# kkahatapitiya/Coarse-Fine-Networks

Measured on AMD Instinct MI355X. Metric: clips/sec (fwd+bwd+SGD) x3d_fine X3D-M T=256x224x224, higher is better.
Workload: dtype f32; 1 GPU; x3d_fine X3D-M train step (fwd+loss+bwd+SGD), 8x3x256x224x224 clips per GPU, random-init weights; clips_per_gpu=8, frames=256, parallelism=dp1, launch=eager

## Files before the change

### coarse-fine-networks_amd/csrc/pwfused.hip

```cpp
#include "cfn_common.h"
#include <stdlib.h>

#include "pw_common.h"

typedef float __attribute__((ext_vector_type(4))) pf4;

#define PF_PT 64
#define PF_PITCH 65

struct PfArgs {
    const float* gy; const float* y; const double* gs; const double* gq; const double* gsc;
    const float* w;
    const float* x; const double* pa; const double* pb;
    float* gx; double* gA; double* gB; double* gw;
    const float* acc; int acc_s, acc_Ho, acc_Wo, Hi, Wi, T;
    int N, M, K, Q, nstrips, stages;
};

template <int MTW, int NTW, int ACT>
__global__ __launch_bounds__(256, ACT < 0 ? 3 : 2) void pw_bwd_fused_kernel(const PfArgs a) {
    extern __shared__ __attribute__((aligned(16))) float smem[];
    constexpr bool EPI = ACT >= 0;
    constexpr int ACTV = EPI ? ACT : CFN_ACT_NONE;
    constexpr int BM = 32 * MTW, BN = 32 * NTW;
    constexpr int NG = BM / 16, NX = BN / 16;
    constexpr int NT16 = BN / 16, KS = BM / 4;
    const int tid = threadIdx.x, wave = tid >> 6, lane = tid & 63, half = lane >> 5, col = lane & 31;
    const int m16 = lane & 15, kq = lane >> 4;
    unsigned L = cfn_xcd_remap(blockIdx.x, gridDim.x);
    const int strip = L % a.nstrips;
    const int n = L / a.nstrips;
    const int M = a.M, K = a.K, Q = a.Q;

    constexpr int IMG = (BM + BN) * PF_PITCH;
    float* img0 = smem;
    float* sCg = smem + 2 * IMG;
    float* sCz = sCg + 2 * BM;
    float* sCx = sCz + BM;
    float* sSt = sCx + 2 * BN;
    for (int m = tid; m < BM; m += 256) {
        const bool ok = m < M;
        sCg[2 * m] = (ok && a.gs) ? (float)a.gs[(long)n * M + m] : 0.0f;
        sCg[2 * m + 1] = (ok && a.gq && a.y) ? 2.0f * (float)a.gq[(long)n * M + m] : 0.0f;
        sCz[m] = (ok && a.gsc) ? (float)a.gsc[(long)n * M + m] : 1.0f;
    }
    for (int k = tid; k < BN; k += 256) {
        const bool ok = EPI && k < K;
        sCx[2 * k] = ok ? (float)a.pa[(long)n * K + k] : 1.0f;
        sCx[2 * k + 1] = ok ? (float)a.pb[(long)n * K + k] : 0.0f;
    }
    float wq[NT16][KS];
#pragma unroll
    for (int t = 0; t < NT16; ++t)
#pragma unroll
        for (int s = 0; s < KS; ++s) {
            const int ci = t * 16 + m16, co = 4 * s + kq;
            wq[t][s] = (ci < K && co < M) ? a.w[(long)co * K + ci] : 0.0f;
        }
    float ca[NTW], cb[NTW];
#pragma unroll
    for (int j = 0; j < NTW; ++j) {
        const int k = j * 32 + col;
        const bool ok = EPI && k < K;
        ca[j] = ok ? (float)a.pa[(long)n * K + k] : 1.0f;
        cb[j] = ok ? (float)a.pb[(long)n * K + k] : 0.0f;
    }
    f16v acc[MTW][NTW];
#pragma unroll
    for (int i = 0; i < MTW; ++i)
#pragma unroll
        for (int j = 0; j < NTW; ++j)
#pragma unroll
            for (int r = 0; r < 16; ++r) acc[i][j][r] = 0.0f;
    float sa[NT16][4], sb[NT16][4];
#pragma unroll
    for (int t = 0; t < NT16; ++t)
#pragma unroll
        for (int r = 0; r < 4; ++r) { sa[t][r] = 0.0f; sb[t][r] = 0.0f; }
    __syncthreads();

    const int lrow = tid >> 4, c4 = (tid & 15) * 4;
    constexpr int OOB = 0x7ffffff0;
    __amdgpu_buffer_rsrc_t rg = cfn_rsrc(const_cast<float*>(a.gy + (long)n * M * Q), (unsigned)((long)M * Q * 4));
    __amdgpu_buffer_rsrc_t ry = cfn_rsrc(const_cast<float*>((a.y ? a.y : a.gy) + (long)n * M * Q), a.y ? (unsigned)((long)M * Q * 4) : 0u);
    __amdgpu_buffer_rsrc_t rx = cfn_rsrc(const_cast<float*>(a.x + (long)n * K * Q), (unsigned)((long)K * Q * 4));
    __amdgpu_buffer_rsrc_t rd = cfn_rsrc(a.gx + (long)n * K * Q, (unsigned)((long)K * Q * 4));
    pf4 pg[NG], py[NG], px[NX];
    int vog[NG], vox[NX];
#pragma unroll
    for (int it = 0; it < NG; ++it) vog[it] = (it * 16 + lrow) < M ? ((it * 16 + lrow) * Q + c4) * 4 : OOB;
#pragma unroll
    for (int it = 0; it < NX; ++it) vox[it] = (it * 16 + lrow) < K ? ((it * 16 + lrow) * Q + c4) * 4 : OOB;
    auto prefetch = [&](int q0) {
        const bool inq = q0 + c4 < Q;
#pragma unroll
        for (int it = 0; it < NG; ++it) {
            const int vo = inq ? vog[it] : OOB;
            pg[it] = __builtin_bit_cast(pf4, __builtin_amdgcn_raw_buffer_load_b128(rg, vo, q0 * 4, 0));
            py[it] = __builtin_bit_cast(pf4, __builtin_amdgcn_raw_buffer_load_b128(ry, vo, q0 * 4, 0));
        }
#pragma unroll
        for (int it = 0; it < NX; ++it)
            px[it] = __builtin_bit_cast(pf4, __builtin_amdgcn_raw_buffer_load_b128(rx, inq ? vox[it] : OOB, q0 * 4, 0));
    };
    auto stage = [&](int q0, float* sG, float* sX) {
        const bool inq = q0 + c4 < Q;
#pragma unroll
        for (int it = 0; it < NG; ++it) {
            const int row = it * 16 + lrow;
            const float cs = cfn_settle(sCg[2 * row]), cq = cfn_settle(sCg[2 * row + 1]), cz = cfn_settle(sCz[row]);
            const bool ok = inq && (row < M);
            float* d = sG + row * PF_PITCH + c4;
            d[0] = ok ? fmaf(py[it].x, cq, fmaf(pg[it].x, cz, cs)) : 0.0f;
            d[1] = ok ? fmaf(py[it].y, cq, fmaf(pg[it].y, cz, cs)) : 0.0f;
            d[2] = ok ? fmaf(py[it].z, cq, fmaf(pg[it].z, cz, cs)) : 0.0f;
            d[3] = ok ? fmaf(py[it].w, cq, fmaf(pg[it].w, cz, cs)) : 0.0f;
        }
#pragma unroll
        for (int it = 0; it < NX; ++it) {
            const int row = it * 16 + lrow;
            float* d = sX + row * PF_PITCH + c4;
            d[0] = px[it].x; d[1] = px[it].y; d[2] = px[it].z; d[3] = px[it].w;
        }
    };

    const int qbeg = strip * a.stages * PF_PT;
    const int nst = min(a.stages, (Q - qbeg + PF_PT - 1) / PF_PT);
    if (nst > 0) {
        prefetch(qbeg);
        stage(qbeg, img0, img0 + BM * PF_PITCH);
        if (nst > 1) prefetch(qbeg + PF_PT);
    }
    __syncthreads();
    const int pbase = wave * (PF_PT / 4);
    const int hw = a.Hi * a.Wi;
    const int acc_pitch4 = a.T * a.acc_Ho * a.acc_Wo * 4;
    __amdgpu_buffer_rsrc_t racc = cfn_rsrc(const_cast<float*>(a.acc ? a.acc + (long)n * K * (acc_pitch4 / 4) : a.gy), a.acc ? (unsigned)((long)K * acc_pitch4) : 0u);
    for (int st = 0; st < nst; ++st) {
        const int q0 = qbeg + st * PF_PT;
        float* cur = img0 + (st & 1) * IMG;
        float* nxt = img0 + ((st + 1) & 1) * IMG;
        if (st + 1 < nst) {
            stage(q0 + PF_PT, nxt, nxt + BM * PF_PITCH);
            if (st + 2 < nst) prefetch(q0 + 2 * PF_PT);
        }
        const float* sG = cur;
        const float* sX = cur + BM * PF_PITCH;
#pragma unroll
        for (int s = 0; s < PF_PT / 8; ++s) {
            const int p = pbase + 2 * s + half;
            float av[MTW], bv[NTW];
#pragma unroll
            for (int i = 0; i < MTW; ++i) av[i] = sG[(i * 32 + col) * PF_PITCH + p];
#pragma unroll
            for (int j = 0; j < NTW; ++j) {
                const float xr = sX[(j * 32 + col) * PF_PITCH + p];
                bv[j] = EPI ? cfn_act<ACTV>(fmaf(xr, ca[j], cb[j])) : xr;
            }
#pragma unroll
            for (int i = 0; i < MTW; ++i)
#pragma unroll
                for (int j = 0; j < NTW; ++j) acc[i][j] = __builtin_amdgcn_mfma_f32_32x32x2f32(av[i], bv[j], acc[i][j], 0, 0, 0);
        }
        pf4 da[NT16];
#pragma unroll
        for (int t = 0; t < NT16; ++t) da[t] = (pf4){0.f, 0.f, 0.f, 0.f};
#pragma unroll
        for (int s = 0; s < KS; ++s) {
            const float b = sG[(4 * s + kq) * PF_PITCH + pbase + m16];
#pragma unroll
            for (int t = 0; t < NT16; ++t) da[t] = __builtin_amdgcn_mfma_f32_16x16x4f32(wq[t][s], b, da[t], 0, 0, 0);
        }
        const int q = q0 + pbase + m16;
        const bool qv = q < Q;
        int aoff = OOB;
        if (a.acc && qv) {
            const int tq = q / hw, rq = q - tq * hw;
            const int hq = rq / a.Wi, wq_ = rq - hq * a.Wi;
            if (hq % a.acc_s == 0 && wq_ % a.acc_s == 0) aoff = (((tq * a.acc_Ho + hq / a.acc_s) * a.acc_Wo + wq_ / a.acc_s)) * 4;
        }
        float av4[NT16][4];
#pragma unroll
        for (int t = 0; t < NT16; ++t)
#pragma unroll
            for (int r = 0; r < 4; ++r) av4[t][r] = 0.0f;
        if (a.acc) {
            const unsigned arow = (unsigned)aoff + (unsigned)(4 * kq) * (unsigned)acc_pitch4;
#pragma unroll
            for (int t = 0; t < NT16; ++t)
#pragma unroll
                for (int r = 0; r < 4; ++r)
                    av4[t][r] = __builtin_bit_cast(float, __builtin_amdgcn_raw_buffer_load_b32(
                        racc, (int)(aoff == OOB ? (unsigned)OOB : arow + (unsigned)r * (unsigned)acc_pitch4), t * 16 * acc_pitch4, 0));
        }
#pragma unroll
        for (int t = 0; t < NT16; ++t) {
#pragma unroll
            for (int r = 0; r < 4; ++r) {
                const int ci = t * 16 + 4 * kq + r;
                const bool ok = qv && ci < K;
                float v = da[t][r] + av4[t][r];
                if (EPI) {
                    const float xr = sX[ci * PF_PITCH + pbase + m16];
                    const float pa = sCx[2 * ci], pb = sCx[2 * ci + 1];
                    const float dz = ok ? v * cfn_act_grad<ACTV>(fmaf(xr, pa, pb)) : 0.0f;
                    sa[t][r] = fmaf(dz, xr, sa[t][r]);
                    sb[t][r] += dz;
                    v = dz * pa;
                }
                __builtin_amdgcn_raw_buffer_store_b32(__builtin_bit_cast(unsigned, v), rd, ok ? (ci * Q + pbase + m16) * 4 : OOB, q0 * 4, 0);
            }
        }
        __syncthreads();
    }

    if (EPI) {
#pragma unroll
        for (int t = 0; t < NT16; ++t)
#pragma unroll
            for (int r = 0; r < 4; ++r) {
                float u = sa[t][r], v = sb[t][r];
#pragma unroll
                for (int o = 1; o < 16; o <<= 1) { u += __shfl_xor(u, o, 64); v += __shfl_xor(v, o, 64); }
                if (m16 == 0) {
                    const int ci = t * 16 + 4 * kq + r;
                    sSt[(wave * BN + ci) * 2] = u;
                    sSt[(wave * BN + ci) * 2 + 1] = v;
                }
            }
    }
    constexpr int CWP = BN + 1;
    float* cw = smem + wave * (BM * CWP);
#pragma unroll
    for (int i = 0; i < MTW; ++i)
#pragma unroll
        for (int j = 0; j < NTW; ++j)
#pragma unroll
            for (int r = 0; r < 16; ++r) {
                const int ml = i * 32 + (r & 3) + 8 * (r >> 2) + 4 * half;
                cw[ml * CWP + j * 32 + col] = acc[i][j][r];
            }
    __syncthreads();
    for (int e = tid; e < BM * BN; e += 256) {
        const int ml = e / BN, kl = e - ml * BN;
        const int o = ml * CWP + kl;
        const float v = (smem[o] + smem[BM * CWP + o]) + (smem[2 * BM * CWP + o] + smem[3 * BM * CWP + o]);
        if (ml < M && kl < K) cfn_add64(&a.gw[(long)ml * K + kl], (double)v);
    }
    if (EPI && tid < K) {
        const float u = (sSt[2 * tid] + sSt[(BN + tid) * 2]) + (sSt[(2 * BN + tid) * 2] + sSt[(3 * BN + tid) * 2]);
        const float v = (sSt[2 * tid + 1] + sSt[(BN + tid) * 2 + 1]) + (sSt[(2 * BN + tid) * 2 + 1] + sSt[(3 * BN + tid) * 2 + 1]);
        cfn_add64(&a.gA[(long)n * K + tid], (double)u);
        cfn_add64(&a.gB[(long)n * K + tid], (double)v);
    }
}

template <int MTW, int NTW>
static int pf_launch(const PfArgs& a, int act, bool epi, unsigned blocks, hipStream_t st) {
    constexpr int BM = 32 * MTW, BN = 32 * NTW;
    size_t lds = ((size_t)2 * (BM + BN) * PF_PITCH + 3 * BM + 10 * BN) * sizeof(float);
    const size_t lds_cw = (size_t)4 * BM * (BN + 1) * sizeof(float);
    if (lds_cw > lds) lds = lds_cw;
#define CFN_PF_GO(ACTV)                                                                                         \
    do {                                                                                                        \
        auto k = pw_bwd_fused_kernel<MTW, NTW, ACTV>;                                                           \
        if (lds > 48 * 1024) (void)hipFuncSetAttribute((const void*)k, hipFuncAttributeMaxDynamicSharedMemorySize, (int)lds); \
        hipLaunchKernelGGL(k, dim3(blocks), dim3(256), lds, st, a);                                             \
    } while (0)
    if (!epi) CFN_PF_GO(-1);
    else if (act == CFN_ACT_RELU) CFN_PF_GO(CFN_ACT_RELU);
    else if (act == CFN_ACT_SWISH) CFN_PF_GO(CFN_ACT_SWISH);
    else CFN_PF_GO(CFN_ACT_NONE);
#undef CFN_PF_GO
    return cfn_check_launch("pwconv_bwd_fused");
}

extern "C" int cfn_pwconv_bwd_fused(const float* gy, const float* y, const double* gsum, const double* gsumsq, const float* w,
                                    const float* x, const double* A, const double* B, int act, float* gx, double* gA, double* gB,
                                    double* gw, int N, int Cin, int Cout, int T, int Hi, int Wi, const float* acc, int acc_stride,
                                    const double* gscale, void* stream) {
    CFN_REQUIRE(gy && w && x && gx && gw, "cfn_pwconv_bwd_fused: null tensor");
    CFN_REQUIRE((A == nullptr) == (B == nullptr), "cfn_pwconv_bwd_fused: A/B mismatch");
    CFN_REQUIRE(A == nullptr || (gA && gB), "cfn_pwconv_bwd_fused: prologue needs gA, gB");
    CFN_REQUIRE(gsumsq == nullptr || y != nullptr, "cfn_pwconv_bwd_fused: gsumsq needs y");
    CFN_REQUIRE(acc == nullptr || acc_stride >= 1, "cfn_pwconv_bwd_fused: bad acc_stride");
    {
        const int rs = pwfs_try_launch(gy, y, gsum, gsumsq, w, x, A, B, act, gx, gA, gB, gw, N, Cin, Cout, T, Hi, Wi, acc, acc_stride, gscale, (hipStream_t)stream);
        if (rs != -1) return rs;
    }
    const long Ql = (long)T * Hi * Wi;
    if (Cin > 64 || Cout > 64 || (Cin > 32 && Cout > 32) || Ql % 4 != 0 || Ql >= (1L << 30)) return -1;
    if ((long)Cout * Ql * 4 >= 0x7ffffff0L || (long)Cin * Ql * 4 >= 0x7ffffff0L) return -1;
    if (A && act != CFN_ACT_NONE && act != CFN_ACT_RELU && act != CFN_ACT_SWISH) return -1;
    if ((((uintptr_t)gy | (uintptr_t)x | (uintptr_t)(y ? y : gy)) & 15) != 0) return -1;
    PfArgs a = {};
    a.gy = gy; a.y = gsumsq ? y : nullptr; a.gs = gsum; a.gq = gsumsq; a.gsc = gscale; a.w = w; a.x = x; a.pa = A; a.pb = B;
    a.gx = gx; a.gA = gA; a.gB = gB; a.gw = gw;
    a.acc = acc; a.acc_s = acc ? acc_stride : 1; a.Hi = Hi; a.Wi = Wi; a.T = T;
    a.acc_Ho = (Hi - 1) / a.acc_s + 1; a.acc_Wo = (Wi - 1) / a.acc_s + 1;
    a.N = N; a.M = Cout; a.K = Cin; a.Q = (int)Ql;
    const long nst = cfn_cdiv(Ql, PF_PT);
    const bool epi = A != nullptr;
    long want = (epi ? 1024 : 1536) / N;
    if (want < 1) want = 1;
    long stages = cfn_cdiv(nst, want);
    if (stages < 4) stages = 4;
    a.stages = (int)stages;
    a.nstrips = (int)cfn_cdiv(nst, stages);
    const unsigned blocks = (unsigned)((long)N * a.nstrips);
    hipStream_t st = (hipStream_t)stream;
    CfnProfScope prof(CFN_K_PWCONV_BWD, st, 4.0 * N * ((double)Cout * Ql * (a.y ? 2 : 1) + (double)Cin * Ql * 2));
    if (Cout > 32) return pf_launch<2, 1>(a, act, epi, blocks, st);
    if (Cin > 32) return pf_launch<1, 2>(a, act, epi, blocks, st);
    return pf_launch<1, 1>(a, act, epi, blocks, st);
}
```

Before: 107.0 clips/s.

## Add warp-specialized 512-thread pointwise-conv backward kernel splitting dW and dX waves

Adds a 512-thread variant of the fused pointwise-conv backward kernel. Four waves stage data and accumulate the weight gradient while four other waves compute the input gradient and activation epilogue, with weights held in LDS for wider tiles and the acc loads issued early. It is used for epilogue cases whose tile exceeds 32x32, so the two GEMM-like tasks can overlap on separate waves. Debug knockout switches are compiled in only under a macro. The cost is more LDS and registers per block, extra synchronisation, and lower occupancy per block.

New measurement: 107.5 clips/s, median of 6. About the same (+0.5%).

```diff
diff --git a/coarse-fine-networks_amd/csrc/pwfused.hip b/coarse-fine-networks_amd/csrc/pwfused.hip
--- a/coarse-fine-networks_amd/csrc/pwfused.hip
+++ b/coarse-fine-networks_amd/csrc/pwfused.hip
@@ -15,7 +15,15 @@
     float* gx; double* gA; double* gB; double* gw;
     const float* acc; int acc_s, acc_Ho, acc_Wo, Hi, Wi, T;
     int N, M, K, Q, nstrips, stages;
+#ifdef CFN_PWF_KNOCKOUTS
+    int dbg;
+#endif
 };
+#ifdef CFN_PWF_KNOCKOUTS
+#define PF_DBG(a) ((a).dbg)
+#else
+#define PF_DBG(a) 0
+#endif
 
 template <int MTW, int NTW, int ACT>
 __global__ __launch_bounds__(256, ACT < 0 ? 3 : 2) void pw_bwd_fused_kernel(const PfArgs a) {
@@ -146,6 +154,7 @@
         }
         const float* sG = cur;
         const float* sX = cur + BM * PF_PITCH;
+        if (!(PF_DBG(a) & 1))
 #pragma unroll
         for (int s = 0; s < PF_PT / 8; ++s) {
             const int p = pbase + 2 * s + half;
@@ -165,6 +174,7 @@
         pf4 da[NT16];
 #pragma unroll
         for (int t = 0; t < NT16; ++t) da[t] = (pf4){0.f, 0.f, 0.f, 0.f};
+        if (!(PF_DBG(a) & 2))
 #pragma unroll
         for (int s = 0; s < KS; ++s) {
             const float b = sG[(4 * s + kq) * PF_PITCH + pbase + m16];
@@ -200,7 +210,7 @@
                 const int ci = t * 16 + 4 * kq + r;
                 const bool ok = qv && ci < K;
                 float v = da[t][r] + av4[t][r];
-                if (EPI) {
+                if (EPI && !(PF_DBG(a) & 4)) {
                     const float xr = sX[ci * PF_PITCH + pbase + m16];
                     const float pa = sCx[2 * ci], pb = sCx[2 * ci + 1];
                     const float dz = ok ? v * cfn_act_grad<ACTV>(fmaf(xr, pa, pb)) : 0.0f;
@@ -208,7 +218,7 @@
                     sb[t][r] += dz;
                     v = dz * pa;
                 }
-                __builtin_amdgcn_raw_buffer_store_b32(__builtin_bit_cast(unsigned, v), rd, ok ? (ci * Q + pbase + m16) * 4 : OOB, q0 * 4, 0);
+                __builtin_amdgcn_raw_buffer_store_b32(__builtin_bit_cast(unsigned, v), rd, (ok && !(PF_DBG(a) & 8)) ? (ci * Q + pbase + m16) * 4 : OOB, q0 * 4, 0);
             }
         }
         __syncthreads();
@@ -255,23 +265,334 @@
     }
 }
 
+template <int MTW, int NTW, int ACT>
+__global__ __launch_bounds__(512, 4) void pw_bwd_fused8_kernel(const PfArgs a) {
+    extern __shared__ __attribute__((aligned(16))) float smem[];
+    constexpr bool EPI = ACT >= 0;
+    constexpr int ACTV = EPI ? ACT : CFN_ACT_NONE;
+    constexpr int BM = 32 * MTW, BN = 32 * NTW;
+    constexpr int NG = BM / 16, NX = BN / 16;
+    constexpr int NT16 = BN / 16, KS = BM / 4;
+    constexpr bool WLDS = NT16 > 2;
+    const int tid = threadIdx.x, wave = tid >> 6, lane = tid & 63, half = lane >> 5, col = lane & 31;
+    const int m16 = lane & 15, kq = lane >> 4, w4 = wave & 3;
+    unsigned L = cfn_xcd_remap(blockIdx.x, gridDim.x);
+    const int strip = L % a.nstrips;
+    const int n = L / a.nstrips;
+    const int M = a.M, K = a.K, Q = a.Q;
+
+    constexpr int IMG = (BM + BN) * PF_PITCH;
+    float* img0 = smem;
+    float* sCg = smem + 2 * IMG;
+    float* sCz = sCg + 2 * BM;
+    float* sCx = sCz + BM;
+    float* sSt = sCx + 2 * BN;
+    float* sWt = sSt + 8 * BN;
+    for (int m = tid; m < BM; m += 512) {
+        const bool ok = m < M;
+        sCg[2 * m] = (ok && a.gs) ? (float)a.gs[(long)n * M + m] : 0.0f;
+        sCg[2 * m + 1] = (ok && a.gq && a.y) ? 2.0f * (float)a.gq[(long)n * M + m] : 0.0f;
+        sCz[m] = (ok && a.gsc) ? (float)a.gsc[(long)n * M + m] : 1.0f;
+    }
+    for (int k = tid; k < BN; k += 512) {
+        const bool ok = EPI && k < K;
+        sCx[2 * k] = ok ? (float)a.pa[(long)n * K + k] : 1.0f;
+        sCx[2 * k + 1] = ok ? (float)a.pb[(long)n * K + k] : 0.0f;
+    }
+    __syncthreads();
+
+    constexpr int OOB = 0x7ffffff0;
+    const int qbeg = strip * a.stages * PF_PT;
+    const int nst = min(a.stages, (Q - qbeg + PF_PT - 1) / PF_PT);
+    const int pbase = w4 * (PF_PT / 4);
+    constexpr int CWP = BN + 1;
+
+    if (wave < 4) {
+        float ca[NTW], cb[NTW];
+#pragma unroll
+        for (int j = 0; j < NTW; ++j) {
+            const int k = j * 32 + col;
+            const bool ok = EPI && k < K;
+            ca[j] = ok ? (float)a.pa[(long)n * K + k] : 1.0f;
+            cb[j] = ok ? (float)a.pb[(long)n * K + k] : 0.0f;
+        }
+        f16v acc[MTW][NTW];
+#pragma unroll
+        for (int i = 0; i < MTW; ++i)
+#pragma unroll
+            for (int j = 0; j < NTW; ++j)
+#pragma unroll
+                for (int r = 0; r < 16; ++r) acc[i][j][r] = 0.0f;
+        const int lrow = tid >> 4, c4 = (tid & 15) * 4;
+        __amdgpu_buffer_rsrc_t rg = cfn_rsrc(const_cast<float*>(a.gy + (long)n * M * Q), (unsigned)((long)M * Q * 4));
+        __amdgpu_buffer_rsrc_t ry = cfn_rsrc(const_cast<float*>((a.y ? a.y : a.gy) + (long)n * M * Q), a.y ? (unsigned)((long)M * Q * 4) : 0u);
+        __amdgpu_buffer_rsrc_t rx = cfn_rsrc(const_cast<float*>(a.x + (long)n * K * Q), (unsigned)((long)K * Q * 4));
+        pf4 pg[NG], py[NG], px[NX];
+        const int vo0 = (lrow * Q + c4) * 4, vstep = 16 * Q * 4;
+        auto prefetch_g = [&](int q0) {
+            const bool inq = q0 + c4 < Q;
+#pragma unroll
+            for (int it = 0; it < NG; ++it) {
+                const int vo = (inq && it * 16 + lrow < M) ? vo0 + it * vstep : OOB;
+                pg[it] = __builtin_bit_cast(pf4, __builtin_amdgcn_raw_buffer_load_b128(rg, vo, q0 * 4, 0));
+                py[it] = __builtin_bit_cast(pf4, __builtin_amdgcn_raw_buffer_load_b128(ry, vo, q0 * 4, 0));
+            }
+        };
+        auto prefetch_x = [&](int q0) {
+            const bool inq = q0 + c4 < Q;
+#pragma unroll
+            for (int it = 0; it < NX; ++it)
+                px[it] = __builtin_bit_cast(pf4, __builtin_amdgcn_raw_buffer_load_b128(rx, (inq && it * 16 + lrow < K) ? vo0 + it * vstep : OOB, q0 * 4, 0));
+        };
+        auto stage_g = [&](int q0, float* sG) {
+            const bool inq = q0 + c4 < Q;
+#pragma unroll
+            for (int it = 0; it < NG; ++it) {
+                const int row = it * 16 + lrow;
+                const float cs = cfn_settle(sCg[2 * row]), cq = cfn_settle(sCg[2 * row + 1]), cz = cfn_settle(sCz[row]);
+                const bool ok = inq && (row < M);
+                float* d = sG + row * PF_PITCH + c4;
+                d[0] = ok ? fmaf(py[it].x, cq, fmaf(pg[it].x, cz, cs)) : 0.0f;
+                d[1] = ok ? fmaf(py[it].y, cq, fmaf(pg[it].y, cz, cs)) : 0.0f;
+                d[2] = ok ? fmaf(py[it].z, cq, fmaf(pg[it].z, cz, cs)) : 0.0f;
+                d[3] = ok ? fmaf(py[it].w, cq, fmaf(pg[it].w, cz, cs)) : 0.0f;
+            }
+        };
+        auto stage_x = [&](float* sX) {
+#pragma unroll
+            for (int it = 0; it < NX; ++it) {
+                float* d = sX + (it * 16 + lrow) * PF_PITCH + c4;
+                d[0] = px[it].x; d[1] = px[it].y; d[2] = px[it].z; d[3] = px[it].w;
+            }
+        };
+        if (nst > 0) {
+            prefetch_x(qbeg);
+            prefetch_g(qbeg);
+            stage_x(img0 + BM * PF_PITCH);
+            if (nst > 1) prefetch_x(qbeg + PF_PT);
+            stage_g(qbeg, img0);
+            if (nst > 1) prefetch_g(qbeg + PF_PT);
+        }
+        __syncthreads();
+        for (int st = 0; st < nst; ++st) {
+            const int q0 = qbeg + st * PF_PT;
+            float* cur = img0 + (st & 1) * IMG;
+            float* nxt = img0 + ((st + 1) & 1) * IMG;
+            if (st + 1 < nst) {
+                stage_x(nxt + BM * PF_PITCH);
+                if (st + 2 < nst) prefetch_x(q0 + 2 * PF_PT);
+                stage_g(q0 + PF_PT, nxt);
+                if (st + 2 < nst) prefetch_g(q0 + 2 * PF_PT);
+            }
+            const float* sG = cur;
+            const float* sX = cur + BM * PF_PITCH;
+            if (!(PF_DBG(a) & 1))
+#pragma unroll
+            for (int s = 0; s < PF_PT / 8; ++s) {
+                const int p = pbase + 2 * s + half;
+                float av[MTW], bv[NTW];
+#pragma unroll
+                for (int i = 0; i < MTW; ++i) av[i] = sG[(i * 32 + col) * PF_PITCH + p];
+#pragma unroll
+                for (int j = 0; j < NTW; ++j) {
+                    const float xr = sX[(j * 32 + col) * PF_PITCH + p];
+                    bv[j] = EPI ? cfn_act<ACTV>(fmaf(xr, ca[j], cb[j])) : xr;
+                }
+#pragma unroll
+                for (int i = 0; i < MTW; ++i)
+#pragma unroll
+                    for (int j = 0; j < NTW; ++j) acc[i][j] = __builtin_amdgcn_mfma_f32_32x32x2f32(av[i], bv[j], acc[i][j], 0, 0, 0);
+            }
+            __syncthreads();
+        }
+        float* cw = smem + wave * (BM * CWP);
+#pragma unroll
+        for (int i = 0; i < MTW; ++i)
+#pragma unroll
+            for (int j = 0; j < NTW; ++j)
+#pragma unroll
+                for (int r = 0; r < 16; ++r) {
+                    const int ml = i * 32 + (r & 3) + 8 * (r >> 2) + 4 * half;
+                    cw[ml * CWP + j * 32 + col] = acc[i][j][r];
+                }
+    } else {
+        float wq[WLDS ? 1 : NT16][WLDS ? 1 : KS];
+        if (WLDS) {
+            if (wave == 4) {
+#pragma unroll
+                for (int t = 0; t < NT16; ++t)
+#pragma unroll
+                    for (int s = 0; s < KS; ++s) {
+                        const int ci = t * 16 + m16, co = 4 * s + kq;
+                        sWt[(((s >> 2) * NT16 + t) * 64 + lane) * 4 + (s & 3)] = (ci < K && co < M) ? a.w[(long)co * K + ci] : 0.0f;
+                    }
+            }
+        } else {
+#pragma unroll
+            for (int t = 0; t < NT16; ++t)
+#pragma unroll
+                for (int s = 0; s < KS; ++s) {
+                    const int ci = t * 16 + m16, co = 4 * s + kq;
+                    wq[t][s] = (ci < K && co < M) ? a.w[(long)co * K + ci] : 0.0f;
+                }
+        }
+        float sa[NT16][4], sb[NT16][4];
+#pragma unroll
+        for (int t = 0; t < NT16; ++t)
+#pragma unroll
+            for (int r = 0; r < 4; ++r) { sa[t][r] = 0.0f; sb[t][r] = 0.0f; }
+        __amdgpu_buffer_rsrc_t rd = cfn_rsrc(a.gx + (long)n * K * Q, (unsigned)((long)K * Q * 4));
+        const int hw = a.Hi * a.Wi;
+        const int acc_pitch4 = a.T * a.acc_Ho * a.acc_Wo * 4;
+        __amdgpu_buffer_rsrc_t racc = cfn_rsrc(const_cast<float*>(a.acc ? a.acc + (long)n * K * (acc_pitch4 / 4) : a.gy), a.acc ? (unsigned)((long)K * acc_pitch4) : 0u);
+        auto acc_off = [&](int q0) {
+            const int q = q0 + pbase + m16;
+            int aoff = OOB;
+            if (a.acc && q < Q) {
+                const int tq = q / hw, rq = q - tq * hw;
+                const int hq = rq / a.Wi, wq_ = rq - hq * a.Wi;
+                if (hq % a.acc_s == 0 && wq_ % a.acc_s == 0) aoff = (((tq * a.acc_Ho + hq / a.acc_s) * a.acc_Wo + wq_ / a.acc_s)) * 4;
+            }
+            return aoff;
+        };
+        auto acc_load = [&](int aoff, int t, float* o) {
+            const unsigned arow = (unsigned)aoff + (unsigned)(4 * kq) * (unsigned)acc_pitch4;
+#pragma unroll
+            for (int r = 0; r < 4; ++r)
+                o[r] = __builtin_bit_cast(float, __builtin_amdgcn_raw_buffer_load_b32(
+                    racc, (int)(aoff == OOB ? (unsigned)OOB : arow + (unsigned)r * (unsigned)acc_pitch4), t * 16 * acc_pitch4, 0));
+        };
+        constexpr bool ACC_EARLY = NT16 <= 2;
+        float avn[NT16][4];
+#pragma unroll
+        for (int t = 0; t < NT16; ++t)
+#pragma unroll
+            for (int r = 0; r < 4; ++r) avn[t][r] = 0.0f;
+        if (ACC_EARLY) {
+            const int ao = acc_off(qbeg);
+#pragma unroll
+            for (int t = 0; t < NT16; ++t) acc_load(ao, t, avn[t]);
+        }
+        __syncthreads();
+        for (int st = 0; st < nst; ++st) {
+            const int q0 = qbeg + st * PF_PT;
+            const float* sG = img0 + (st & 1) * IMG;
+            const float* sX = sG + BM * PF_PITCH;
+            const bool qv = q0 + pbase + m16 < Q;
+            float av4[NT16][4];
+#pragma unroll
+            for (int t = 0; t < NT16; ++t)
+#pragma unroll
+                for (int r = 0; r < 4; ++r) av4[t][r] = avn[t][r];
+            const int aoff = acc_off(ACC_EARLY ? (st + 1 < nst ? q0 + PF_PT : Q) : q0);
+            if (ACC_EARLY) {
+#pragma unroll
+                for (int t = 0; t < NT16; ++t) acc_load(aoff, t, avn[t]);
+            }
+            pf4 da[NT16];
+#pragma unroll
+            for (int t = 0; t < NT16; ++t) da[t] = (pf4){0.f, 0.f, 0.f, 0.f};
+            if (!(PF_DBG(a) & 2)) {
+                if (WLDS) {
+#pragma unroll
+                    for (int g = 0; g < KS / 4; ++g) {
+                        pf4 wv[NT16];
+#pragma unroll
+                        for (int t = 0; t < NT16; ++t) wv[t] = *reinterpret_cast<const pf4*>(sWt + ((g * NT16 + t) * 64 + lane) * 4);
+#pragma unroll
+                        for (int s4 = 0; s4 < 4; ++s4) {
+                            const float b = sG[(4 * (4 * g + s4) + kq) * PF_PITCH + pbase + m16];
+#pragma unroll
+                            for (int t = 0; t < NT16; ++t) da[t] = __builtin_amdgcn_mfma_f32_16x16x4f32(wv[t][s4], b, da[t], 0, 0, 0);
+                        }
+                    }
+                } else {
+#pragma unroll
+                    for (int s = 0; s < KS; ++s) {
+                        const float b = sG[(4 * s + kq) * PF_PITCH + pbase + m16];
+#pragma unroll
+                        for (int t = 0; t < NT16; ++t) da[t] = __builtin_amdgcn_mfma_f32_16x16x4f32(wq[t][s], b, da[t], 0, 0, 0);
+                    }
+                }
+            }
+            const bool epi_on = !(PF_DBG(a) & 4), st_on = !(PF_DBG(a) & 8);
+#pragma unroll
+            for (int t = 0; t < NT16; ++t) {
+                if (!ACC_EARLY && a.acc) acc_load(aoff, t, av4[t]);
+#pragma unroll
+                for (int r = 0; r < 4; ++r) {
+                    const int ci = t * 16 + 4 * kq + r;
+                    const bool ok = qv && ci < K;
+                    float v = da[t][r] + av4[t][r];
+                    if (EPI && epi_on) {
+                        const float xr = sX[ci * PF_PITCH + pbase + m16];
+                        const float pa = sCx[2 * ci], pb = sCx[2 * ci + 1];
+                        const float dz = ok ? v * cfn_act_grad<ACTV>(fmaf(xr, pa, pb)) : 0.0f;
+                        sa[t][r] = fmaf(dz, xr, sa[t][r]);
+                        sb[t][r] += dz;
+                        v = dz * pa;
+                    }
+                    __builtin_amdgcn_raw_buffer_store_b32(__builtin_bit_cast(unsigned, v), rd, (ok && st_on) ? (ci * Q + pbase + m16) * 4 : OOB, q0 * 4, 0);
+                }
+            }
+            __syncthreads();
+        }
+        if (EPI) {
+#pragma unroll
+            for (int t = 0; t < NT16; ++t)
+#pragma unroll
+                for (int r = 0; r < 4; ++r) {
+                    float u = sa[t][r], v = sb[t][r];
+#pragma unroll
+                    for (int o = 1; o < 16; o <<= 1) { u += __shfl_xor(u, o, 64); v += __shfl_xor(v, o, 64); }
+                    if (m16 == 0) {
+                        const int ci = t * 16 + 4 * kq + r;
+                        sSt[(w4 * BN + ci) * 2] = u;
+                        sSt[(w4 * BN + ci) * 2 + 1] = v;
+                    }
+                }
+        }
+    }
+    __syncthreads();
+    for (int e = tid; e < BM * BN; e += 512) {
+        const int ml = e / BN, kl = e - ml * BN;
+        const int o = ml * CWP + kl;
+        const float v = (smem[o] + smem[BM * CWP + o]) + (smem[2 * BM * CWP + o] + smem[3 * BM * CWP + o]);
+        if (ml < M && kl < K) cfn_add64(&a.gw[(long)ml * K + kl], (double)v);
+    }
+    if (EPI && tid < K) {
+        const float u = (sSt[2 * tid] + sSt[(BN + tid) * 2]) + (sSt[(2 * BN + tid) * 2] + sSt[(3 * BN + tid) * 2]);
+        const float v = (sSt[2 * tid + 1] + sSt[(BN + tid) * 2 + 1]) + (sSt[(2 * BN + tid) * 2 + 1] + sSt[(3 * BN + tid) * 2 + 1]);
+        cfn_add64(&a.gA[(long)n * K + tid], (double)u);
+        cfn_add64(&a.gB[(long)n * K + tid], (double)v);
+    }
+}
+
+template <int MTW, int NTW> constexpr int pf_mode(bool epi) { return (epi && MTW + NTW > 2) ? 1 : 0; }
+
 template <int MTW, int NTW>
-static int pf_launch(const PfArgs& a, int act, bool epi, unsigned blocks, hipStream_t st) {
+static int pf_launch(const PfArgs& a, int act, bool epi, int mode, unsigned blocks, hipStream_t st) {
     constexpr int BM = 32 * MTW, BN = 32 * NTW;
-    size_t lds = ((size_t)2 * (BM + BN) * PF_PITCH + 3 * BM + 10 * BN) * sizeof(float);
+    size_t lds = ((size_t)2 * (BM + BN) * PF_PITCH + 3 * BM + 10 * BN + (mode && BN > 32 ? BM * BN : 0)) * sizeof(float);
     const size_t lds_cw = (size_t)4 * BM * (BN + 1) * sizeof(float);
     if (lds_cw > lds) lds = lds_cw;
+#define CFN_PF_GO1(KERNEL, THREADS)                                                                             \
+    do {                                                                                                        \
+        auto k = KERNEL;                                                                                        \
+        if (lds > 48 * 1024) (void)hipFuncSetAttribute((const void*)k, hipFuncAttributeMaxDynamicSharedMemorySize, (int)lds); \
+        hipLaunchKernelGGL(k, dim3(blocks), dim3(THREADS), lds, st, a);                                         \
+    } while (0)
 #define CFN_PF_GO(ACTV)                                                                                         \
     do {                                                                                                        \
-        auto k = pw_bwd_fused_kernel<MTW, NTW, ACTV>;                                                           \
-        if (lds > 48 * 1024) (void)hipFuncSetAttribute((const void*)k, hipFuncAttributeMaxDynamicSharedMemorySize, (int)lds); \
-        hipLaunchKernelGGL(k, dim3(blocks), dim3(256), lds, st, a);                                             \
+        if (mode == 1) CFN_PF_GO1((pw_bwd_fused8_kernel<MTW, NTW, ACTV>), 512);                                 \
+        else CFN_PF_GO1((pw_bwd_fused_kernel<MTW, NTW, ACTV>), 256);                                            \
     } while (0)
     if (!epi) CFN_PF_GO(-1);
     else if (act == CFN_ACT_RELU) CFN_PF_GO(CFN_ACT_RELU);
     else if (act == CFN_ACT_SWISH) CFN_PF_GO(CFN_ACT_SWISH);
     else CFN_PF_GO(CFN_ACT_NONE);
 #undef CFN_PF_GO
+#undef CFN_PF_GO1
     return cfn_check_launch("pwconv_bwd_fused");
 }
 
@@ -299,9 +620,19 @@
     a.acc = acc; a.acc_s = acc ? acc_stride : 1; a.Hi = Hi; a.Wi = Wi; a.T = T;
     a.acc_Ho = (Hi - 1) / a.acc_s + 1; a.acc_Wo = (Wi - 1) / a.acc_s + 1;
     a.N = N; a.M = Cout; a.K = Cin; a.Q = (int)Ql;
+    const bool epi = A != nullptr;
+    int mode = Cout > 32 ? pf_mode<2, 1>(epi) : Cin > 32 ? pf_mode<1, 2>(epi) : pf_mode<1, 1>(epi);
+#ifdef CFN_PWF_KNOCKOUTS
+    const char* ko_env = getenv("CFN_PWFS_DBG");
+    const int ko = ko_env ? atoi(ko_env) : 0;
+    a.dbg = ko & 15;
+    if ((ko >> 4) & 3) mode = ((ko >> 4) & 3) == 1 ? 0 : 1;
+#endif
     const long nst = cfn_cdiv(Ql, PF_PT);
-    const bool epi = A != nullptr;
-    long want = (epi ? 1024 : 1536) / N;
+    long want = (mode == 0 && !epi ? 1536 : 1024) / N;
+#ifdef CFN_PWF_KNOCKOUTS
+    if (ko >> 8) want = (ko >> 8) / N;
+#endif
     if (want < 1) want = 1;
     long stages = cfn_cdiv(nst, want);
     if (stages < 4) stages = 4;
@@ -310,7 +641,7 @@
     const unsigned blocks = (unsigned)((long)N * a.nstrips);
     hipStream_t st = (hipStream_t)stream;
     CfnProfScope prof(CFN_K_PWCONV_BWD, st, 4.0 * N * ((double)Cout * Ql * (a.y ? 2 : 1) + (double)Cin * Ql * 2));
-    if (Cout > 32) return pf_launch<2, 1>(a, act, epi, blocks, st);
-    if (Cin > 32) return pf_launch<1, 2>(a, act, epi, blocks, st);
-    return pf_launch<1, 1>(a, act, epi, blocks, st);
+    if (Cout > 32) return pf_launch<2, 1>(a, act, epi, mode, blocks, st);
+    if (Cin > 32) return pf_launch<1, 2>(a, act, epi, mode, blocks, st);
+    return pf_launch<1, 1>(a, act, epi, mode, blocks, st);
 }
```
